# volume-em/empanada

Measured on AMD Instinct MI355X. Metric: Mvox/s end-to-end 3D panoptic inference (incl. consensus); PQ vs CPU ref, higher is better.
Workload: dtype f32

## Files before the change

### empanada_amd/csrc/emp_conv.hip

```cpp
#include "emp_common.h"
#include <stdlib.h>

typedef float f32x16 __attribute__((ext_vector_type(16)));

#define CG_BM 128
#define CG_BK 32
#define CG_THREADS 256

struct ConvGeom {
    const float *x, *w, *scale, *shift, *res;
    float *out;
    int N, H, W, Cin, OH, OW, Cout, KH, KW, stride, pad, dil, relu;
    int64_t M, out_ps, res_ps;
    int tiles_m, tiles_n;
    int64_t x_bs, w_bs, out_bs;
    const int32_t *tiles;
    const float *proj_w;
    float *proj_out;
    int proj_n;
    int64_t hw;
};

__device__ __attribute__((aligned(16))) float cg_zero_page[64];

// ... 408 lines not shown
                        *reinterpret_cast<float4 *>(g.out + p * g.out_ps + co) = make_float4(v[0], v[1], v[2], v[3]);
                    } else {
#pragma unroll
                        for (int e = 0; e < 4; ++e)
                            if (co + e < g.Cout) g.out[p * g.out_ps + co + e] = v[e];
                    }
                }
            }
            if constexpr (PROJ) {
                float ps[4] = {0.f, 0.f, 0.f, 0.f};
                if (valid && co + 3 < g.Cout) {
#pragma unroll
                    for (int q = 0; q < 4; ++q)
                        if (q < g.proj_n) {
                            const float4 wq = *reinterpret_cast<const float4 *>(g.proj_w + (int64_t)q * g.Cout + co);
                            ps[q] = __fadd_rn(__fadd_rn(__fadd_rn(__fmul_rn(v[0], wq.x), __fmul_rn(v[1], wq.y)),
                                                        __fmul_rn(v[2], wq.z)), __fmul_rn(v[3], wq.w));
                        }
                }
                *reinterpret_cast<float4 *>(&Cs[lrow_c * CLD + ccol]) = make_float4(ps[0], ps[1], ps[2], ps[3]);
            }
        }
        if constexpr (PROJ) {
            __syncthreads();
            for (int idx = tid; idx < EPI_ROWS * g.proj_n; idx += CG_THREADS) {
                const int row_l = idx / g.proj_n, q = idx - row_l * g.proj_n;
                const int64_t p = m0 + rd * EPI_ROWS + row_l;
                if (p < g.M) {
                    float t = Cs[row_l * CLD + q];
#pragma unroll 8
                    for (int j = 1; j < C4; ++j) t = __fadd_rn(t, Cs[row_l * CLD + 4 * j + q]);
                    const int64_t img = p / g.hw;
                    atomicAdd(g.proj_out + (img * g.proj_n + q) * g.hw + (p - img * g.hw), t);
                }
            }
        }
    }
}

struct CgPlan {
    bool narrow, respf, glds;
    int slab, tiles_m, tiles_n;
};

static CgPlan cg_plan(int64_t M, int Cout, int batch, bool has_res, bool res_vec_ok, bool may_split_n = true, int cin = 32)
{
    CgPlan p;
    const int64_t wide_blocks = emp_cdiv(M, CG_BM) * emp_cdiv(Cout, 128) * batch;
    p.narrow = Cout <= 64 || (Cout % 128 != 0 && Cout % 128 <= 64 && Cout < 512) || (may_split_n && wide_blocks < 256);
    p.tiles_m = (int)emp_cdiv(M, CG_BM);
    p.tiles_n = (int)emp_cdiv(Cout, p.narrow ? 64 : 128);
    static const char *fnarrow = getenv("EMP_CONV_NARROW");
    static const char *norespf = getenv("EMP_CONV_NO_RESPF");
    if (fnarrow && fnarrow[0] == '1') {
        p.narrow = true;
        p.tiles_n = (int)emp_cdiv(Cout, 64);
    }
    p.respf = has_res && res_vec_ok && Cout % (p.narrow ? 64 : 128) == 0 && !norespf;
    static const char *force = getenv("EMP_CONV_BK");
    const int64_t blocks = (int64_t)p.tiles_m * p.tiles_n * batch;
    p.slab = blocks > 512 ? 16 : 32;
    if (force && force[0] == '1') p.slab = 16;
    if (force && force[0] == '3') p.slab = 32;
    if (p.respf) p.slab = 32;
    if (cin % 32 != 0) {
        p.slab = 16;
        p.respf = false;
    }
    static const char *noglds = getenv("EMP_CONV_NO_GLDS");
    p.glds = !noglds;
    return p;
}

extern "C" int emp_conv_k_slab(int64_t M, int Cout, int batch, int has_residual)
{
    return cg_plan(M, Cout, batch, has_residual != 0, true).slab;
}

extern "C" int emp_conv_k_slab_cin(int64_t M, int Cout, int batch, int has_residual, int Cin)
{
    return cg_plan(M, Cout, batch, has_residual != 0, true, true, Cin).slab;
}

extern "C" int emp_conv1x1_ws_eligible(int64_t M, int Cin, int Cout, int KH, int KW, int stride, int pad, int relu);
extern "C" __attribute__((visibility("hidden"))) int emp_conv1x1_ws_launch(const float *x, const float *w, const float *scale, const float *shift,
                                     const float *res, int64_t res_ps, int relu, int64_t M, int Cin, int Cout,
                                     float *out, int64_t out_ps, void *stream);

extern "C" int emp_conv_k_slab_geom(int64_t M, int Cout, int has_residual, int Cin, int KH, int KW, int stride, int pad,
                                    int relu)
{
    if (emp_conv1x1_ws_eligible(M, Cin, Cout, KH, KW, stride, pad, relu)) return 64;
    return cg_plan(M, Cout, 1, has_residual != 0 && relu != 2, true, true, Cin).slab;
}

extern "C" int emp_conv_bn_act_nhwc(const float *x, const float *w_okkc, const float *scale, const float *shift,
                                    const float *residual, int64_t res_pixel_stride, int relu, int N, int H, int W,
                                    int Cin, int Cout, int KH, int KW, int stride, int pad, int dil, float *out,
                                    int64_t out_pixel_stride, void *stream)
{
    EMP_REQUIRE(x && w_okkc && out, "conv: null pointer");
    EMP_REQUIRE(N >= 0 && H > 0 && W > 0 && Cin > 0 && Cout > 0, "conv: bad shape");
    EMP_REQUIRE(Cin % 16 == 0, "conv: Cin %d must be a multiple of 16", Cin);
    EMP_REQUIRE(relu != 2 || residual, "conv: the gate epilogue (relu == 2) needs the gated tensor as residual");
    EMP_REQUIRE(KH >= 1 && KW >= 1 && KH <= 7 && KW <= 7 && stride >= 1 && dil >= 1 && pad >= 0, "conv: bad filter geometry");
    const int OH = (H + 2 * pad - dil * (KH - 1) - 1) / stride + 1;
    const int OW = (W + 2 * pad - dil * (KW - 1) - 1) / stride + 1;
    EMP_REQUIRE(OH > 0 && OW > 0, "conv: empty output");
    if (out_pixel_stride == 0) out_pixel_stride = Cout;
    if (res_pixel_stride == 0) res_pixel_stride = Cout;
    EMP_REQUIRE(out_pixel_stride >= Cout && res_pixel_stride >= Cout, "conv: bad pixel stride");
    EMP_REQUIRE(((reinterpret_cast<uintptr_t>(x) | reinterpret_cast<uintptr_t>(w_okkc)) & 15) == 0,
                "conv: x and w must be 16-byte aligned");
    EMP_REQUIRE(out != x, "conv: output cannot alias the input");
    if (N == 0) return EMP_OK;
    ConvGeom g;
    g.x = x; g.w = w_okkc; g.scale = scale; g.shift = shift; g.res = residual; g.out = out;
    g.N = N; g.H = H; g.W = W; g.Cin = Cin; g.OH = OH; g.OW = OW; g.Cout = Cout; g.KH = KH; g.KW = KW;
    g.stride = stride; g.pad = pad; g.dil = dil; g.relu = relu;
    g.M = (int64_t)N * OH * OW; g.out_ps = out_pixel_stride; g.res_ps = res_pixel_stride;
    g.x_bs = g.w_bs = g.out_bs = 0; g.tiles = nullptr; g.proj_w = nullptr; g.proj_out = nullptr; g.proj_n = 0; g.hw = 1;
    const bool res_vec_ok = (res_pixel_stride & 3) == 0 && (reinterpret_cast<uintptr_t>(residual) & 15) == 0;
    const bool io_vec_ok = res_vec_ok && (out_pixel_stride & 3) == 0 && (reinterpret_cast<uintptr_t>(out) & 15) == 0 &&
                           (!scale || (reinterpret_cast<uintptr_t>(scale) & 15) == 0) &&
                           (!shift || (reinterpret_cast<uintptr_t>(shift) & 15) == 0);
    if (io_vec_ok && scale && shift && emp_conv1x1_ws_eligible(g.M, Cin, Cout, KH, KW, stride, pad, relu))
        return emp_conv1x1_ws_launch(x, w_okkc, scale, shift, residual, res_pixel_stride, relu, g.M, Cin, Cout, out,
                                     out_pixel_stride, stream);
    const CgPlan pl = cg_plan(g.M, Cout, 1, residual != nullptr && relu != 2, res_vec_ok, true, Cin);
    const bool narrow = pl.narrow, respf = pl.respf, bk16 = pl.slab == 16;
    EMP_REQUIRE((int64_t)pl.tiles_m * pl.tiles_n < (1LL << 28), "conv: too many tiles");
    g.tiles_m = pl.tiles_m;
    g.tiles_n = pl.tiles_n;
    const int T = g.tiles_m * g.tiles_n;
    const int grid = 8 * ((T + 7) / 8);
#define CG_GO(NT_, RES_, BK_, GL_) hipLaunchKernelGGL((conv_igemm_f32_kernel<NT_, 0, RES_, BK_, false, GL_>), dim3(grid), dim3(CG_THREADS), 0, emp_stream(stream), g)
#define CG_GATE(NT_, BK_) hipLaunchKernelGGL((conv_igemm_f32_kernel<NT_, 0, false, BK_, false, true, true>), dim3(grid), dim3(CG_THREADS), 0, emp_stream(stream), g)
    if (relu == 2) {
        if (narrow) { if (bk16) CG_GATE(1, 16); else CG_GATE(1, 32); }
        else { if (bk16) CG_GATE(2, 16); else CG_GATE(2, 32); }
    } else if (narrow) {
        if (respf) { if (pl.glds) CG_GO(1, true, 32, true); else CG_GO(1, true, 32, false); }
        else if (pl.glds) { if (bk16) CG_GO(1, false, 16, true); else CG_GO(1, false, 32, true); }
        else { if (bk16) CG_GO(1, false, 16, false); else CG_GO(1, false, 32, false); }
    } else {
        if (respf) { if (pl.glds) CG_GO(2, true, 32, true); else CG_GO(2, true, 32, false); }
        else if (pl.glds) { if (bk16) CG_GO(2, false, 16, true); else CG_GO(2, false, 32, true); }
        else { if (bk16) CG_GO(2, false, 16, false); else CG_GO(2, false, 32, false); }
    }
#undef CG_GO
#undef CG_GATE
    EMP_CHECK_LAUNCH("emp_conv_bn_act_nhwc");
    return EMP_OK;
}

__global__ __launch_bounds__(256) void splitk_reduce_kernel(const float *__restrict__ work, int nz, int64_t M, int Cout,
                                                            const float *__restrict__ scale,
                                                            const float *__restrict__ shift,
                                                            const float *__restrict__ res, int64_t res_ps, int relu,
                                                            float *__restrict__ out, int64_t out_ps)
{
    const int C4 = Cout >> 2;
    const int64_t total = M * C4, plane = M * (int64_t)Cout;
    for (int64_t i = (int64_t)blockIdx.x * blockDim.x + threadIdx.x; i < total; i += (int64_t)gridDim.x * blockDim.x) {
        const int64_t p = i / C4;
        const int co = (int)(i - p * C4) * 4;
        const float *w = work + p * Cout + co;
        float4 t = *reinterpret_cast<const float4 *>(w);
        for (int z = 1; z < nz; ++z) {
            const float4 u = *reinterpret_cast<const float4 *>(w + z * plane);
            t.x = __fadd_rn(t.x, u.x); t.y = __fadd_rn(t.y, u.y); t.z = __fadd_rn(t.z, u.z); t.w = __fadd_rn(t.w, u.w);
        }
        float v[4] = {t.x, t.y, t.z, t.w};
#pragma unroll
        for (int e = 0; e < 4; ++e) {
            const float sc = scale ? scale[co + e] : 1.f, sh = shift ? shift[co + e] : 0.f;
            v[e] = __fadd_rn(__fmul_rn(v[e], sc), sh);
        }
        if (res) {
            const float4 r4 = *reinterpret_cast<const float4 *>(res + p * res_ps + co);
            v[0] = __fadd_rn(v[0], r4.x); v[1] = __fadd_rn(v[1], r4.y); v[2] = __fadd_rn(v[2], r4.z); v[3] = __fadd_rn(v[3], r4.w);
        }
        if (relu) {
#pragma unroll
            for (int e = 0; e < 4; ++e) v[e] = fmaxf(v[e], 0.f);
        }
        *reinterpret_cast<float4 *>(out + p * out_ps + co) = make_float4(v[0], v[1], v[2], v[3]);
    }
}

extern "C" int emp_conv_splitk_plan(int64_t M, int Cout, int Cin, int KH, int KW)
{
    if (M <= 0 || Cout <= 0 || Cin % 32 != 0 || Cout % 4 != 0) return 1;
    const CgPlan pl = cg_plan(M, Cout, 1, false, true, true, Cin);
    const int64_t tiles = (int64_t)pl.tiles_m * pl.tiles_n;
    const int S = KH * KW * (Cin / 32);
    if (tiles > 128) return 1;
    int64_t k = 256 / tiles;
    if (k > S / 4) k = S / 4;
    if (k > 32) k = 32;
    return k >= 2 ? (int)k : 1;
}

extern "C" int emp_conv_splitk_bn_act_nhwc(const float *x, const float *w_okkc, const float *scale, const float *shift,
                                           const float *residual, int64_t res_pixel_stride, int relu, int N, int H, int W,
                                           int Cin, int Cout, int KH, int KW, int stride, int pad, int dil, int k_splits,
                                           float *work, float *out, int64_t out_pixel_stride, void *stream)
{
    EMP_REQUIRE(x && w_okkc && out && work, "conv_splitk: null pointer");
    EMP_REQUIRE(N >= 0 && H > 0 && W > 0 && Cin > 0 && Cout > 0, "conv_splitk: bad shape");
    EMP_REQUIRE(Cin % 32 == 0 && Cout % 4 == 0, "conv_splitk: Cin %d must be a multiple of 32, Cout %d of 4", Cin, Cout);
    EMP_REQUIRE(relu == 0 || relu == 1, "conv_splitk: relu must be 0 or 1");
// ... 112 lines not shown
            dst[(1 * 4 + v) * ps] = W_ADD(tt[1][v], tt[2][v]);
            dst[(2 * 4 + v) * ps] = W_SUB(tt[2][v], tt[1][v]);
            dst[(3 * 4 + v) * ps] = W_SUB(tt[1][v], tt[3][v]);
        }
    }
}

__global__ __launch_bounds__(256) void wino_output_kernel(const float4 *__restrict__ Mw, const int32_t *__restrict__ tiles,
                                                          int64_t T, int H, int W, int Co4, int dil,
                                                          const float4 *__restrict__ scale, const float4 *__restrict__ shift,
                                                          int relu, float *__restrict__ out, int64_t out_ps)
{
    const int64_t total = T * Co4;
    for (int64_t i = (int64_t)blockIdx.x * blockDim.x + threadIdx.x; i < total; i += (int64_t)gridDim.x * blockDim.x) {
        const int c4 = (int)(i % Co4);
        const int64_t t = i / Co4;
        const int n = tiles[3 * t], oy = tiles[3 * t + 1] + dil, ox = tiles[3 * t + 2] + dil;
        const float4 *src = Mw + t * Co4 + c4;
        const int64_t ps = T * Co4;
        float4 m[4][4];
#pragma unroll
        for (int a = 0; a < 4; ++a)
#pragma unroll
            for (int b = 0; b < 4; ++b) m[a][b] = src[(a * 4 + b) * ps];
        float4 s[2][4];
#pragma unroll
        for (int b = 0; b < 4; ++b) {
            s[0][b] = W_ADD(W_ADD(m[0][b], m[1][b]), m[2][b]);
            s[1][b] = W_SUB(W_SUB(m[1][b], m[2][b]), m[3][b]);
        }
        float4 sc = make_float4(1.f, 1.f, 1.f, 1.f), sh = make_float4(0.f, 0.f, 0.f, 0.f);
        if (scale) sc = scale[c4];
        if (shift) sh = shift[c4];
#pragma unroll
        for (int a = 0; a < 2; ++a) {
            float4 yv[2];
            yv[0] = W_ADD(W_ADD(s[a][0], s[a][1]), s[a][2]);
            yv[1] = W_SUB(W_SUB(s[a][1], s[a][2]), s[a][3]);
#pragma unroll
            for (int b = 0; b < 2; ++b) {
                const int yy = oy + a * dil, xx = ox + b * dil;
                if (yy < H && xx < W) {
                    float4 v = yv[b];
                    if (scale) v = make_float4(__fmul_rn(v.x, sc.x), __fmul_rn(v.y, sc.y), __fmul_rn(v.z, sc.z), __fmul_rn(v.w, sc.w));
                    if (shift) v = W_ADD(v, sh);
                    if (relu) v = make_float4(fmaxf(v.x, 0.f), fmaxf(v.y, 0.f), fmaxf(v.z, 0.f), fmaxf(v.w, 0.f));
                    *reinterpret_cast<float4 *>(out + (((int64_t)n * H + yy) * W + xx) * out_ps + 4 * c4) = v;
                }
            }
        }
    }
}
#undef W_SUB
#undef W_ADD

extern "C" int emp_wino_input_transform(const float *x, int N, int H, int W, int C, int dil, const int32_t *tiles,
                                        int64_t T, float *V, void *stream)
{
    EMP_REQUIRE(x && tiles && V, "wino_input: null pointer");
    EMP_REQUIRE(N > 0 && H > 0 && W > 0 && C > 0 && C % 4 == 0 && dil >= 1 && T >= 0, "wino_input: bad shape");
    EMP_REQUIRE(((reinterpret_cast<uintptr_t>(x) | reinterpret_cast<uintptr_t>(V)) & 15) == 0, "wino_input: alignment");
    if (T == 0) return EMP_OK;
    hipLaunchKernelGGL(wino_input_kernel, dim3(emp_grid(T * (C / 4), 256, 16384)), dim3(256), 0, emp_stream(stream), x,
                       tiles, T, H, W, C / 4, dil, reinterpret_cast<float4 *>(V));
    EMP_CHECK_LAUNCH("emp_wino_input_transform");
    return EMP_OK;
}

extern "C" int emp_gemm_nt_batched(const float *A, const float *B, int batch, int64_t M, int N, int K, float *C,
                                   void *stream)
{
    EMP_REQUIRE(A && B && C, "gemm: null pointer");
    EMP_REQUIRE(batch >= 1 && batch <= 65535 && M >= 0 && M < (1LL << 31) && N > 0 && K > 0 && K % CG_BK == 0,
                "gemm: bad shape (K must be a multiple of %d)", CG_BK);
    EMP_REQUIRE(((reinterpret_cast<uintptr_t>(A) | reinterpret_cast<uintptr_t>(B)) & 15) == 0, "gemm: alignment");
    if (M == 0) return EMP_OK;
    ConvGeom g;
    g.x = A; g.w = B; g.scale = g.shift = g.res = nullptr; g.out = C;
    g.N = 1; g.H = 1; g.W = (int)M; g.Cin = K; g.OH = 1; g.OW = (int)M; g.Cout = N; g.KH = g.KW = 1;
    g.stride = 1; g.pad = 0; g.dil = 1; g.relu = 0;
    g.M = M; g.out_ps = N; g.res_ps = N;
    g.x_bs = M * K; g.w_bs = (int64_t)N * K; g.out_bs = M * N; g.tiles = nullptr; g.proj_w = nullptr; g.proj_out = nullptr; g.proj_n = 0; g.hw = 1;
    const CgPlan pl = cg_plan(M, N, batch, false, true);
    const bool narrow = pl.narrow, bk16 = pl.slab == 16;
    g.tiles_m = pl.tiles_m;
    g.tiles_n = pl.tiles_n;
    const int T = g.tiles_m * g.tiles_n;
    dim3 grid(8 * ((T + 7) / 8), batch);
#define CG_GOG(NT_, BK_, GL_) hipLaunchKernelGGL((conv_igemm_f32_kernel<NT_, 0, false, BK_, false, GL_>), grid, dim3(CG_THREADS), 0, emp_stream(stream), g)
    if (narrow) {
        if (pl.glds) { if (bk16) CG_GOG(1, 16, true); else CG_GOG(1, 32, true); }
        else { if (bk16) CG_GOG(1, 16, false); else CG_GOG(1, 32, false); }
    } else {
        if (pl.glds) { if (bk16) CG_GOG(2, 16, true); else CG_GOG(2, 32, true); }
        else { if (bk16) CG_GOG(2, 16, false); else CG_GOG(2, 32, false); }
    }
#undef CG_GOG
    EMP_CHECK_LAUNCH("emp_gemm_nt_batched");
    return EMP_OK;
}

extern "C" int emp_wino_gemm_fused(const float *x, int N, int H, int W, int Cin, int dil, const int32_t *tiles,
                                   int64_t T, const float *U, int Cout, float *Mw, void *stream)
{
    EMP_REQUIRE(x && tiles && U && Mw, "wino_gemm: null pointer");
    EMP_REQUIRE(N > 0 && H > 0 && W > 0 && Cin > 0 && Cin % CG_BK == 0 && Cout > 0 && dil >= 1 && T >= 0,
                "wino_gemm: bad shape (Cin must be a multiple of %d)", CG_BK);
    EMP_REQUIRE((int64_t)N * H * W * Cin < (1LL << 31) && T < (1LL << 31), "wino_gemm: activation too large for 32-bit offsets");
    EMP_REQUIRE(((reinterpret_cast<uintptr_t>(x) | reinterpret_cast<uintptr_t>(U)) & 15) == 0, "wino_gemm: alignment");
    if (T == 0) return EMP_OK;
    ConvGeom g;
    g.x = x; g.w = U; g.scale = g.shift = g.res = nullptr; g.out = Mw;
    g.N = N; g.H = H; g.W = W; g.Cin = Cin; g.OH = 1; g.OW = 1; g.Cout = Cout; g.KH = g.KW = 1;
    g.stride = 1; g.pad = 0; g.dil = dil; g.relu = 0;
    g.M = T; g.out_ps = Cout; g.res_ps = Cout;
    g.x_bs = 0; g.w_bs = (int64_t)Cout * Cin; g.out_bs = T * Cout; g.tiles = tiles; g.proj_w = nullptr; g.proj_out = nullptr; g.proj_n = 0; g.hw = 1;
    const bool narrow = Cout <= 64;
    g.tiles_m = (int)emp_cdiv(T, CG_BM);
    g.tiles_n = (int)emp_cdiv(Cout, narrow ? 64 : 128);
    const int nt = g.tiles_m * g.tiles_n;
    dim3 grid(8 * ((nt + 7) / 8), 16);
    if (narrow) hipLaunchKernelGGL((conv_igemm_f32_kernel<1, 1>), grid, dim3(CG_THREADS), 0, emp_stream(stream), g);
    else hipLaunchKernelGGL((conv_igemm_f32_kernel<2, 1>), grid, dim3(CG_THREADS), 0, emp_stream(stream), g);
    EMP_CHECK_LAUNCH("emp_wino_gemm_fused");
    return EMP_OK;
}

extern "C" int emp_wino_output_transform(const float *Mw, const int32_t *tiles, int64_t T, int N, int H, int W,
                                         int Cout, int dil, const float *scale, const float *shift, int relu,
                                         float *out, int64_t out_pixel_stride, void *stream)
{
    EMP_REQUIRE(Mw && tiles && out, "wino_output: null pointer");
    EMP_REQUIRE(N > 0 && H > 0 && W > 0 && Cout > 0 && Cout % 4 == 0 && dil >= 1 && T >= 0, "wino_output: bad shape");
    if (out_pixel_stride == 0) out_pixel_stride = Cout;
    EMP_REQUIRE(out_pixel_stride >= Cout && out_pixel_stride % 4 == 0, "wino_output: bad pixel stride");
    EMP_REQUIRE(((reinterpret_cast<uintptr_t>(Mw) | reinterpret_cast<uintptr_t>(out) | reinterpret_cast<uintptr_t>(scale) |
                  reinterpret_cast<uintptr_t>(shift)) & 15) == 0, "wino_output: alignment");
    if (T == 0) return EMP_OK;
    hipLaunchKernelGGL(wino_output_kernel, dim3(emp_grid(T * (Cout / 4), 256, 16384)), dim3(256), 0, emp_stream(stream),
                       reinterpret_cast<const float4 *>(Mw), tiles, T, H, W, Cout / 4, dil,
                       reinterpret_cast<const float4 *>(scale), reinterpret_cast<const float4 *>(shift), relu, out,
                       out_pixel_stride);
    EMP_CHECK_LAUNCH("emp_wino_output_transform");
    return EMP_OK;
}

struct v4 {
    float x, y, z, w;
};
__device__ __forceinline__ v4 operator+(v4 a, v4 b) { return {__fadd_rn(a.x, b.x), __fadd_rn(a.y, b.y), __fadd_rn(a.z, b.z), __fadd_rn(a.w, b.w)}; }
__device__ __forceinline__ v4 operator-(v4 a, v4 b) { return {__fsub_rn(a.x, b.x), __fsub_rn(a.y, b.y), __fsub_rn(a.z, b.z), __fsub_rn(a.w, b.w)}; }
__device__ __forceinline__ v4 operator*(float k, v4 a) { return {__fmul_rn(k, a.x), __fmul_rn(k, a.y), __fmul_rn(k, a.z), __fmul_rn(k, a.w)}; }
__device__ __forceinline__ v4 ldv4(const float4 *p) { float4 t = *p; return {t.x, t.y, t.z, t.w}; }
__device__ __forceinline__ void stv4(float4 *p, v4 a) { *p = make_float4(a.x, a.y, a.z, a.w); }

__device__ __forceinline__ void wino4_bt(const v4 d[6], v4 r[6])
{
    r[0] = (4.f * d[0] - 5.f * d[2]) + d[4];
    r[1] = (d[3] + d[4]) - 4.f * (d[1] + d[2]);
    r[2] = (d[4] - d[3]) + 4.f * (d[1] - d[2]);
    r[3] = (d[4] - d[2]) + 2.f * (d[3] - d[1]);
    r[4] = (d[4] - d[2]) + 2.f * (d[1] - d[3]);
    r[5] = (4.f * d[1] - 5.f * d[3]) + d[5];
}

__device__ __forceinline__ void wino4_at(const v4 m[6], v4 s[4])
// ... 262 lines not shown
```

### empanada_amd/csrc/emp_conv1x1.hip

```cpp
#include "emp_common.h"
#include <stdlib.h>

typedef float f32x16 __attribute__((ext_vector_type(16)));

#define PW_THREADS 256
#define PW_BN 128
#define PW_ROWS 32

struct PwGeom {
    const float *x, *w, *scale, *shift, *res;
    float *out;
    int64_t M, out_ps, res_ps;
    int Cin, Cout, relu, groups, pix_blocks;
};

template <int KS, bool RES, bool RELU>
__global__ __launch_bounds__(PW_THREADS, 1) void conv1x1_ws_kernel(PwGeom g)
{
    constexpr int CIN = 64 * KS;
    constexpr int LD = CIN + 4;
    __shared__ __attribute__((aligned(16))) float Bs[PW_BN * LD];

    const int bid = blockIdx.x;
    const int xcd = bid & 7, slot = bid >> 3;
    const int per_xcd = g.pix_blocks >> 3;
    const int gi = slot % g.groups;
    const int pb = xcd * per_xcd + slot / g.groups;
    const int n0 = gi * PW_BN;
    const int tid = threadIdx.x;

    for (int idx = tid; idx < PW_BN * (CIN / 4); idx += PW_THREADS) {
        const int rr = idx / (CIN / 4), k4 = idx - rr * (CIN / 4);
        const int co = n0 + 4 * (rr & 31) + (rr >> 5);
        *reinterpret_cast<float4 *>(&Bs[rr * LD + 4 * k4]) = *reinterpret_cast<const float4 *>(g.w + (int64_t)co * CIN + 4 * k4);
    }
    __syncthreads();

    const int wave = tid >> 6, lane = tid & 63;
    const int r = lane & 31, hh = lane >> 5;
    const int co = n0 + 4 * r;
    float sc[4], sh[4];
    { const float4 t = *reinterpret_cast<const float4 *>(g.scale + co); sc[0] = t.x; sc[1] = t.y; sc[2] = t.z; sc[3] = t.w; }
    { const float4 t = *reinterpret_cast<const float4 *>(g.shift + co); sh[0] = t.x; sh[1] = t.y; sh[2] = t.z; sh[3] = t.w; }

    const int64_t n_tiles = (g.M + PW_ROWS - 1) / PW_ROWS;
    const int64_t stride_t = (int64_t)g.pix_blocks * (PW_THREADS / 64);
    const float *Bl = &Bs[r * LD + hh * 32];

    auto load_a = [&](int64_t t, float4 (&a)[KS][8]) {
        const int64_t pa = t * PW_ROWS + r;
        const float *ap = g.x + pa * CIN + hh * 32;
#pragma unroll
        for (int s = 0; s < KS; ++s)
#pragma unroll
            for (int q = 0; q < 8; ++q) a[s][q] = *reinterpret_cast<const float4 *>(ap + 64 * s + 4 * q);
    };
    auto load_rs = [&](int64_t t, float4 (&rs)[RES ? 16 : 1]) {
        if constexpr (RES) {
            const float *rp = g.res + (t * PW_ROWS + 4 * hh) * g.res_ps + co;
#pragma unroll
            for (int q = 0; q < 16; ++q)
                rs[q] = *reinterpret_cast<const float4 *>(rp + (int64_t)((q & 3) + 8 * (q >> 2)) * g.res_ps);
        }
    };
    auto mma = [&](f32x16 (&acc)[4], const float4 (&a)[KS][8]) {
#pragma unroll
        for (int j = 0; j < 4; ++j)
#pragma unroll
            for (int q = 0; q < 16; ++q) acc[j][q] = 0.f;
        int opaque = 0;
        asm volatile("" : "+v"(opaque));
        const float *Bt = Bl + opaque;
#pragma unroll
        for (int s = 0; s < KS; ++s)
#pragma unroll
            for (int q = 0; q < 8; ++q) {
                float4 b[4];
#pragma unroll
                for (int j = 0; j < 4; ++j) b[j] = *reinterpret_cast<const float4 *>(Bt + j * 32 * LD + 64 * s + 4 * q);
#pragma unroll
                for (int e = 0; e < 4; ++e) {
                    const float av = e == 0 ? a[s][q].x : e == 1 ? a[s][q].y : e == 2 ? a[s][q].z : a[s][q].w;
#pragma unroll
                    for (int j = 0; j < 4; ++j) {
                        const float bv = e == 0 ? b[j].x : e == 1 ? b[j].y : e == 2 ? b[j].z : b[j].w;
                        acc[j] = __builtin_amdgcn_mfma_f32_32x32x2f32(av, bv, acc[j], 0, 0, 0);
                    }
                }
            }
    };
    auto outv = [&](const f32x16 (&acc)[4], const float4 (&rs)[RES ? 16 : 1], int q) {
        float v[4] = {acc[0][q], acc[1][q], acc[2][q], acc[3][q]};
#pragma unroll
        for (int e = 0; e < 4; ++e) v[e] = __fadd_rn(__fmul_rn(v[e], sc[e]), sh[e]);
        if constexpr (RES) {
            v[0] = __fadd_rn(v[0], rs[q].x); v[1] = __fadd_rn(v[1], rs[q].y);
            v[2] = __fadd_rn(v[2], rs[q].z); v[3] = __fadd_rn(v[3], rs[q].w);
        }
        if constexpr (RELU) {
#pragma unroll
            for (int e = 0; e < 4; ++e) v[e] = fmaxf(v[e], 0.f);
        }
        return make_float4(v[0], v[1], v[2], v[3]);
    };
    auto epi = [&](const f32x16 (&acc)[4], const float4 (&rs)[RES ? 16 : 1], int64_t t) {
        float *op = g.out + (t * PW_ROWS + 4 * hh) * g.out_ps + co;
#pragma unroll
        for (int q = 0; q < 16; ++q)
            *reinterpret_cast<float4 *>(op + (int64_t)((q & 3) + 8 * (q >> 2)) * g.out_ps) = outv(acc, rs, q);
    };

    const int64_t n_full = g.M / PW_ROWS;
    const int64_t t_first = (int64_t)pb * (PW_THREADS / 64) + wave;
    if (t_first < n_full) {
        const int64_t m = (n_full - t_first + stride_t - 1) / stride_t;
        auto tile = [&](int64_t i) { return t_first + (i < m ? i : m - 1) * stride_t; };
        float4 a0[KS][8], a1[KS][8], rs0[RES ? 16 : 1], rs1[RES ? 16 : 1];
        f32x16 acc0[4], acc1[4];
        load_a(tile(0), a0);
        load_rs(tile(0), rs0);
        load_a(tile(1), a1);
        mma(acc0, a0);
        int64_t i = 1;
        for (; i + 1 < m; i += 2) {
            load_rs(tile(i), rs1);
            load_a(tile(i + 1), a0);
            mma(acc1, a1);
            epi(acc0, rs0, tile(i - 1));
            load_rs(tile(i + 1), rs0);
            load_a(tile(i + 2), a1);
            mma(acc0, a0);
            epi(acc1, rs1, tile(i));
        }
        if (i < m) {
            load_rs(tile(i), rs1);
            mma(acc1, a1);
            epi(acc0, rs0, tile(i - 1));
            epi(acc1, rs1, tile(i));
        } else {
            epi(acc0, rs0, tile(i - 1));
        }
    }
    if (n_full < n_tiles && (n_full - t_first) % stride_t == 0 && n_full >= t_first) {
        const int64_t p0 = n_full * PW_ROWS;
        const int64_t pa = (p0 + r < g.M) ? p0 + r : g.M - 1;
        const float *ap = g.x + pa * CIN + hh * 32;
        float4 a[KS][8], rs[RES ? 16 : 1];
        f32x16 acc[4];
#pragma unroll
        for (int s = 0; s < KS; ++s)
#pragma unroll
            for (int q = 0; q < 8; ++q) a[s][q] = *reinterpret_cast<const float4 *>(ap + 64 * s + 4 * q);
        if constexpr (RES) {
#pragma unroll
            for (int q = 0; q < 16; ++q) {
                int64_t p = p0 + (q & 3) + 8 * (q >> 2) + 4 * hh;
                p = p < g.M ? p : g.M - 1;
                rs[q] = *reinterpret_cast<const float4 *>(g.res + p * g.res_ps + co);
            }
        }
        mma(acc, a);
#pragma unroll
        for (int q = 0; q < 16; ++q) {
            const int64_t p = p0 + (q & 3) + 8 * (q >> 2) + 4 * hh;
            if (p < g.M) *reinterpret_cast<float4 *>(g.out + p * g.out_ps + co) = outv(acc, rs, q);
        }
    }
}

extern "C" int emp_conv1x1_ws_eligible(int64_t M, int Cin, int Cout, int KH, int KW, int stride, int pad, int relu)
{
    static const char *off = getenv("EMP_CONV_NO_WS");
    if (off && off[0] == '1') return 0;
    return KH == 1 && KW == 1 && stride == 1 && pad == 0 && (Cin == 64 || Cin == 128) && Cout % PW_BN == 0 &&
           Cout / PW_BN <= 8 && relu != 2 && M >= 65536;
}

extern "C" __attribute__((visibility("hidden"))) int emp_conv1x1_ws_launch(const float *x, const float *w, const float *scale, const float *shift,
                                     const float *res, int64_t res_ps, int relu, int64_t M, int Cin, int Cout,
                                     float *out, int64_t out_ps, void *stream)
{
    PwGeom g;
    g.x = x; g.w = w; g.scale = scale; g.shift = shift; g.res = res; g.out = out;
    g.M = M; g.out_ps = out_ps; g.res_ps = res_ps; g.Cin = Cin; g.Cout = Cout; g.relu = relu;
    g.groups = Cout / PW_BN;
    int pix = 256 / g.groups;
    pix = pix / 8 * 8;
    if (pix < 8) pix = 8;
    g.pix_blocks = pix;
    const dim3 grid(pix * g.groups), block(PW_THREADS);
    hipStream_t st = emp_stream(stream);
#define PW_GO(KS_, RES_, RELU_) hipLaunchKernelGGL((conv1x1_ws_kernel<KS_, RES_, RELU_>), grid, block, 0, st, g)
#define PW_GO2(KS_, RES_) do { if (relu) PW_GO(KS_, RES_, true); else PW_GO(KS_, RES_, false); } while (0)
    if (Cin == 64) { if (res) PW_GO2(1, true); else PW_GO2(1, false); }
    else { if (res) PW_GO2(2, true); else PW_GO2(2, false); }
#undef PW_GO2
#undef PW_GO
    EMP_CHECK_LAUNCH("emp_conv_bn_act_nhwc(1x1 weight-stationary)");
    return EMP_OK;
}
```

Before: 127.6.

## Extend weight-stationary 1x1 kernel to narrow Cout, wide Cin, and batched GEMM

Generalizes the weight-stationary pointwise MFMA kernel with templated K-slab, Cout tile width (64 or 128) and pixel-tile count. It now covers extra 1x1 conv shapes (256->64, 64->64, 256->128) where the planner picks a 16-wide slab, and the batched NT GEMM path for K and N of 64 or 128. The GEMM mode splits batch×tiles evenly across 256 blocks and restages weights per batch segment. The aim is to replace the generic implicit-GEMM kernel on these large shapes, avoiding repeated weight reloads. The cost is more template instantiations, and K-slab orderings that differ from the old path may slightly change summation order.

Measured after the change: 129.5 (median of 6 runs). 1.02x the previous value.

```diff
diff --git a/empanada_amd/csrc/emp_conv.hip b/empanada_amd/csrc/emp_conv.hip
--- a/empanada_amd/csrc/emp_conv.hip
+++ b/empanada_amd/csrc/emp_conv.hip
@@ -514,15 +514,18 @@
     return cg_plan(M, Cout, batch, has_residual != 0, true, true, Cin).slab;
 }
 
-extern "C" int emp_conv1x1_ws_eligible(int64_t M, int Cin, int Cout, int KH, int KW, int stride, int pad, int relu);
-extern "C" __attribute__((visibility("hidden"))) int emp_conv1x1_ws_launch(const float *x, const float *w, const float *scale, const float *shift,
+extern "C" __attribute__((visibility("hidden"))) int emp_conv1x1_ws_kind(int64_t M, int Cin, int Cout, int KH, int KW, int stride, int pad, int relu);
+extern "C" __attribute__((visibility("hidden"))) int emp_conv1x1_ws_launch(int kind, const float *x, const float *w, const float *scale, const float *shift,
                                      const float *res, int64_t res_ps, int relu, int64_t M, int Cin, int Cout,
                                      float *out, int64_t out_ps, void *stream);
+extern "C" __attribute__((visibility("hidden"))) int emp_gemm_ws_eligible(int batch, int64_t M, int N, int K, int slab);
+extern "C" __attribute__((visibility("hidden"))) int emp_gemm_ws_launch(const float *A, const float *B, int batch, int64_t M, int N, int K, float *C,
+                                                                        void *stream);
 
 extern "C" int emp_conv_k_slab_geom(int64_t M, int Cout, int has_residual, int Cin, int KH, int KW, int stride, int pad,
                                     int relu)
 {
-    if (emp_conv1x1_ws_eligible(M, Cin, Cout, KH, KW, stride, pad, relu)) return 64;
+    if (emp_conv1x1_ws_kind(M, Cin, Cout, KH, KW, stride, pad, relu) == 1) return 64;
     return cg_plan(M, Cout, 1, has_residual != 0 && relu != 2, true, true, Cin).slab;
 }
 
@@ -556,10 +559,14 @@
     const bool io_vec_ok = res_vec_ok && (out_pixel_stride & 3) == 0 && (reinterpret_cast<uintptr_t>(out) & 15) == 0 &&
                            (!scale || (reinterpret_cast<uintptr_t>(scale) & 15) == 0) &&
                            (!shift || (reinterpret_cast<uintptr_t>(shift) & 15) == 0);
-    if (io_vec_ok && scale && shift && emp_conv1x1_ws_eligible(g.M, Cin, Cout, KH, KW, stride, pad, relu))
-        return emp_conv1x1_ws_launch(x, w_okkc, scale, shift, residual, res_pixel_stride, relu, g.M, Cin, Cout, out,
+    const int ws = io_vec_ok && scale && shift ? emp_conv1x1_ws_kind(g.M, Cin, Cout, KH, KW, stride, pad, relu) : 0;
+    if (ws == 1)
+        return emp_conv1x1_ws_launch(1, x, w_okkc, scale, shift, residual, res_pixel_stride, relu, g.M, Cin, Cout, out,
                                      out_pixel_stride, stream);
     const CgPlan pl = cg_plan(g.M, Cout, 1, residual != nullptr && relu != 2, res_vec_ok, true, Cin);
+    if (ws == 2 && !residual && pl.slab == 16)
+        return emp_conv1x1_ws_launch(2, x, w_okkc, scale, shift, nullptr, res_pixel_stride, relu, g.M, Cin, Cout, out,
+                                     out_pixel_stride, stream);
     const bool narrow = pl.narrow, respf = pl.respf, bk16 = pl.slab == 16;
     EMP_REQUIRE((int64_t)pl.tiles_m * pl.tiles_n < (1LL << 28), "conv: too many tiles");
     g.tiles_m = pl.tiles_m;
@@ -838,6 +845,8 @@
     g.M = M; g.out_ps = N; g.res_ps = N;
     g.x_bs = M * K; g.w_bs = (int64_t)N * K; g.out_bs = M * N; g.tiles = nullptr; g.proj_w = nullptr; g.proj_out = nullptr; g.proj_n = 0; g.hw = 1;
     const CgPlan pl = cg_plan(M, N, batch, false, true);
+    if ((reinterpret_cast<uintptr_t>(C) & 15) == 0 && emp_gemm_ws_eligible(batch, M, N, K, pl.slab))
+        return emp_gemm_ws_launch(A, B, batch, M, N, K, C, stream);
     const bool narrow = pl.narrow, bk16 = pl.slab == 16;
     g.tiles_m = pl.tiles_m;
     g.tiles_n = pl.tiles_n;
diff --git a/empanada_amd/csrc/emp_conv1x1.hip b/empanada_amd/csrc/emp_conv1x1.hip
--- a/empanada_amd/csrc/emp_conv1x1.hip
+++ b/empanada_amd/csrc/emp_conv1x1.hip
@@ -4,198 +4,298 @@
 typedef float f32x16 __attribute__((ext_vector_type(16)));
 
 #define PW_THREADS 256
-#define PW_BN 128
 #define PW_ROWS 32
+#define PW_MIN_ROWS 65536
+#define PW_MIN_ROWS_PLAN 262144
 
 struct PwGeom {
     const float *x, *w, *scale, *shift, *res;
     float *out;
     int64_t M, out_ps, res_ps;
     int Cin, Cout, relu, groups, pix_blocks;
+    int batch;
+    int64_t x_bs, w_bs, out_bs;
 };
 
-template <int KS, bool RES, bool RELU>
+template <int KS, int S, int CT, int PT, bool GEMM, bool RES, bool RELU>
 __global__ __launch_bounds__(PW_THREADS, 1) void conv1x1_ws_kernel(PwGeom g)
 {
     constexpr int CIN = 64 * KS;
     constexpr int LD = CIN + 4;
-    __shared__ __attribute__((aligned(16))) float Bs[PW_BN * LD];
+    constexpr int BN = 32 * CT;
+    constexpr int NQ = CIN / 8;
+    constexpr int QS = S / 8;
+    constexpr int ROWS = PW_ROWS * PT;
+    static_assert(!RES || (CT == 4 && PT == 1 && !GEMM), "residual: 128-cout groups of the convolution form only");
+    static_assert(S == 16 || S == 32 || S == 64, "K-slab");
+    __shared__ __attribute__((aligned(16))) float Bs[BN * LD];
 
     const int bid = blockIdx.x;
     const int xcd = bid & 7, slot = bid >> 3;
     const int per_xcd = g.pix_blocks >> 3;
     const int gi = slot % g.groups;
     const int pb = xcd * per_xcd + slot / g.groups;
-    const int n0 = gi * PW_BN;
+    const int n0 = GEMM ? 0 : gi * BN;
     const int tid = threadIdx.x;
-
-    for (int idx = tid; idx < PW_BN * (CIN / 4); idx += PW_THREADS) {
-        const int rr = idx / (CIN / 4), k4 = idx - rr * (CIN / 4);
-        const int co = n0 + 4 * (rr & 31) + (rr >> 5);
-        *reinterpret_cast<float4 *>(&Bs[rr * LD + 4 * k4]) = *reinterpret_cast<const float4 *>(g.w + (int64_t)co * CIN + 4 * k4);
-    }
-    __syncthreads();
+    const float *xb = g.x, *wb = g.w;
+    float *ob = g.out;
+
+    auto stage = [&]() {
+        for (int idx = tid; idx < BN * (CIN / 4); idx += PW_THREADS) {
+            const int rr = idx / (CIN / 4), k4 = idx - rr * (CIN / 4);
+            const int cw = n0 + CT * (rr & 31) + (rr >> 5);
+            *reinterpret_cast<float4 *>(&Bs[rr * LD + 4 * k4]) = *reinterpret_cast<const float4 *>(wb + (int64_t)cw * CIN + 4 * k4);
+        }
+        __syncthreads();
+    };
 
     const int wave = tid >> 6, lane = tid & 63;
     const int r = lane & 31, hh = lane >> 5;
-    const int co = n0 + 4 * r;
-    float sc[4], sh[4];
-    { const float4 t = *reinterpret_cast<const float4 *>(g.scale + co); sc[0] = t.x; sc[1] = t.y; sc[2] = t.z; sc[3] = t.w; }
-    { const float4 t = *reinterpret_cast<const float4 *>(g.shift + co); sh[0] = t.x; sh[1] = t.y; sh[2] = t.z; sh[3] = t.w; }
-
-    const int64_t n_tiles = (g.M + PW_ROWS - 1) / PW_ROWS;
-    const int64_t stride_t = (int64_t)g.pix_blocks * (PW_THREADS / 64);
-    const float *Bl = &Bs[r * LD + hh * 32];
-
-    auto load_a = [&](int64_t t, float4 (&a)[KS][8]) {
-        const int64_t pa = t * PW_ROWS + r;
-        const float *ap = g.x + pa * CIN + hh * 32;
-#pragma unroll
-        for (int s = 0; s < KS; ++s)
-#pragma unroll
-            for (int q = 0; q < 8; ++q) a[s][q] = *reinterpret_cast<const float4 *>(ap + 64 * s + 4 * q);
+    const int co = n0 + CT * r;
+    float sc[CT], sh[CT];
+    if constexpr (!GEMM) {
+        if constexpr (CT == 4) {
+            { const float4 t = *reinterpret_cast<const float4 *>(g.scale + co); sc[0] = t.x; sc[1] = t.y; sc[2] = t.z; sc[3] = t.w; }
+            { const float4 t = *reinterpret_cast<const float4 *>(g.shift + co); sh[0] = t.x; sh[1] = t.y; sh[2] = t.z; sh[3] = t.w; }
+        } else {
+            { const float2 t = *reinterpret_cast<const float2 *>(g.scale + co); sc[0] = t.x; sc[1] = t.y; }
+            { const float2 t = *reinterpret_cast<const float2 *>(g.shift + co); sh[0] = t.x; sh[1] = t.y; }
+        }
+    }
+
+    const int64_t n_tiles = (g.M + ROWS - 1) / ROWS;
+    const int64_t n_full = g.M / ROWS;
+    const float *Bl = &Bs[r * LD + hh * (S / 2)];
+    const int64_t ops = GEMM ? (int64_t)BN : g.out_ps;
+
+    auto load_a = [&](int64_t t, float4 (&a)[PT][NQ]) {
+#pragma unroll
+        for (int p = 0; p < PT; ++p) {
+            const int64_t pa = t * ROWS + PW_ROWS * p + r;
+            const float *ap = xb + pa * CIN + hh * (S / 2);
+#pragma unroll
+            for (int i = 0; i < NQ; ++i) a[p][i] = *reinterpret_cast<const float4 *>(ap + S * (i / QS) + 4 * (i % QS));
+        }
     };
     auto load_rs = [&](int64_t t, float4 (&rs)[RES ? 16 : 1]) {
         if constexpr (RES) {
-            const float *rp = g.res + (t * PW_ROWS + 4 * hh) * g.res_ps + co;
+            const float *rp = g.res + (t * ROWS + 4 * hh) * g.res_ps + co;
 #pragma unroll
             for (int q = 0; q < 16; ++q)
                 rs[q] = *reinterpret_cast<const float4 *>(rp + (int64_t)((q & 3) + 8 * (q >> 2)) * g.res_ps);
         }
     };
-    auto mma = [&](f32x16 (&acc)[4], const float4 (&a)[KS][8]) {
-#pragma unroll
-        for (int j = 0; j < 4; ++j)
+    auto mma = [&](f32x16 (&acc)[PT * CT], const float4 (&a)[PT][NQ]) {
+#pragma unroll
+        for (int j = 0; j < PT * CT; ++j)
 #pragma unroll
             for (int q = 0; q < 16; ++q) acc[j][q] = 0.f;
         int opaque = 0;
         asm volatile("" : "+v"(opaque));
         const float *Bt = Bl + opaque;
 #pragma unroll
-        for (int s = 0; s < KS; ++s)
-#pragma unroll
-            for (int q = 0; q < 8; ++q) {
-                float4 b[4];
-#pragma unroll
-                for (int j = 0; j < 4; ++j) b[j] = *reinterpret_cast<const float4 *>(Bt + j * 32 * LD + 64 * s + 4 * q);
-#pragma unroll
-                for (int e = 0; e < 4; ++e) {
-                    const float av = e == 0 ? a[s][q].x : e == 1 ? a[s][q].y : e == 2 ? a[s][q].z : a[s][q].w;
-#pragma unroll
-                    for (int j = 0; j < 4; ++j) {
+        for (int i = 0; i < NQ; ++i) {
+            float4 b[CT];
+#pragma unroll
+            for (int j = 0; j < CT; ++j) b[j] = *reinterpret_cast<const float4 *>(Bt + j * 32 * LD + S * (i / QS) + 4 * (i % QS));
+#pragma unroll
+            for (int e = 0; e < 4; ++e)
+#pragma unroll
+                for (int p = 0; p < PT; ++p) {
+                    const float av = e == 0 ? a[p][i].x : e == 1 ? a[p][i].y : e == 2 ? a[p][i].z : a[p][i].w;
+#pragma unroll
+                    for (int j = 0; j < CT; ++j) {
                         const float bv = e == 0 ? b[j].x : e == 1 ? b[j].y : e == 2 ? b[j].z : b[j].w;
-                        acc[j] = __builtin_amdgcn_mfma_f32_32x32x2f32(av, bv, acc[j], 0, 0, 0);
+                        acc[p * CT + j] = __builtin_amdgcn_mfma_f32_32x32x2f32(av, bv, acc[p * CT + j], 0, 0, 0);
                     }
                 }
-            }
-    };
-    auto outv = [&](const f32x16 (&acc)[4], const float4 (&rs)[RES ? 16 : 1], int q) {
-        float v[4] = {acc[0][q], acc[1][q], acc[2][q], acc[3][q]};
-#pragma unroll
-        for (int e = 0; e < 4; ++e) v[e] = __fadd_rn(__fmul_rn(v[e], sc[e]), sh[e]);
+        }
+    };
+    auto put = [&](float *dst, const f32x16 (&acc)[PT * CT], int p, const float4 (&rs)[RES ? 16 : 1], int q) {
+        float v[CT];
+#pragma unroll
+        for (int e = 0; e < CT; ++e) v[e] = acc[p * CT + e][q];
+        if constexpr (!GEMM) {
+#pragma unroll
+            for (int e = 0; e < CT; ++e) v[e] = __fadd_rn(__fmul_rn(v[e], sc[e]), sh[e]);
+        }
         if constexpr (RES) {
             v[0] = __fadd_rn(v[0], rs[q].x); v[1] = __fadd_rn(v[1], rs[q].y);
             v[2] = __fadd_rn(v[2], rs[q].z); v[3] = __fadd_rn(v[3], rs[q].w);
         }
         if constexpr (RELU) {
 #pragma unroll
-            for (int e = 0; e < 4; ++e) v[e] = fmaxf(v[e], 0.f);
-        }
-        return make_float4(v[0], v[1], v[2], v[3]);
-    };
-    auto epi = [&](const f32x16 (&acc)[4], const float4 (&rs)[RES ? 16 : 1], int64_t t) {
-        float *op = g.out + (t * PW_ROWS + 4 * hh) * g.out_ps + co;
-#pragma unroll
-        for (int q = 0; q < 16; ++q)
-            *reinterpret_cast<float4 *>(op + (int64_t)((q & 3) + 8 * (q >> 2)) * g.out_ps) = outv(acc, rs, q);
-    };
-
-    const int64_t n_full = g.M / PW_ROWS;
-    const int64_t t_first = (int64_t)pb * (PW_THREADS / 64) + wave;
-    if (t_first < n_full) {
-        const int64_t m = (n_full - t_first + stride_t - 1) / stride_t;
-        auto tile = [&](int64_t i) { return t_first + (i < m ? i : m - 1) * stride_t; };
-        float4 a0[KS][8], a1[KS][8], rs0[RES ? 16 : 1], rs1[RES ? 16 : 1];
-        f32x16 acc0[4], acc1[4];
-        load_a(tile(0), a0);
-        load_rs(tile(0), rs0);
-        load_a(tile(1), a1);
-        mma(acc0, a0);
-        int64_t i = 1;
-        for (; i + 1 < m; i += 2) {
-            load_rs(tile(i), rs1);
-            load_a(tile(i + 1), a0);
-            mma(acc1, a1);
-            epi(acc0, rs0, tile(i - 1));
-            load_rs(tile(i + 1), rs0);
-            load_a(tile(i + 2), a1);
+            for (int e = 0; e < CT; ++e) v[e] = fmaxf(v[e], 0.f);
+        }
+        if constexpr (CT == 4) *reinterpret_cast<float4 *>(dst) = make_float4(v[0], v[1], v[2], v[3]);
+        else *reinterpret_cast<float2 *>(dst) = make_float2(v[0], v[1]);
+    };
+    auto epi = [&](const f32x16 (&acc)[PT * CT], const float4 (&rs)[RES ? 16 : 1], int64_t t) {
+#pragma unroll
+        for (int p = 0; p < PT; ++p) {
+            float *op = ob + (t * ROWS + PW_ROWS * p + 4 * hh) * ops + co;
+#pragma unroll
+            for (int q = 0; q < 16; ++q) put(op + (int64_t)((q & 3) + 8 * (q >> 2)) * ops, acc, p, rs, q);
+        }
+    };
+
+    auto run = [&](const int64_t t_first, const int64_t stride_t, const int64_t t_end) {
+        const int64_t f_end = n_full < t_end ? n_full : t_end;
+        if (t_first < f_end) {
+            const int64_t m = (f_end - t_first + stride_t - 1) / stride_t;
+            auto tile = [&](int64_t i) { return t_first + (i < m ? i : m - 1) * stride_t; };
+            float4 a0[PT][NQ], a1[PT][NQ], rs0[RES ? 16 : 1], rs1[RES ? 16 : 1];
+            f32x16 acc0[PT * CT], acc1[PT * CT];
+            load_a(tile(0), a0);
+            load_rs(tile(0), rs0);
+            load_a(tile(1), a1);
             mma(acc0, a0);
-            epi(acc1, rs1, tile(i));
-        }
-        if (i < m) {
-            load_rs(tile(i), rs1);
-            mma(acc1, a1);
-            epi(acc0, rs0, tile(i - 1));
-            epi(acc1, rs1, tile(i));
-        } else {
-            epi(acc0, rs0, tile(i - 1));
-        }
+            int64_t i = 1;
+            for (; i + 1 < m; i += 2) {
+                load_rs(tile(i), rs1);
+                load_a(tile(i + 1), a0);
+                mma(acc1, a1);
+                epi(acc0, rs0, tile(i - 1));
+                load_rs(tile(i + 1), rs0);
+                load_a(tile(i + 2), a1);
+                mma(acc0, a0);
+                epi(acc1, rs1, tile(i));
+            }
+            if (i < m) {
+                load_rs(tile(i), rs1);
+                mma(acc1, a1);
+                epi(acc0, rs0, tile(i - 1));
+                epi(acc1, rs1, tile(i));
+            } else {
+                epi(acc0, rs0, tile(i - 1));
+            }
+        }
+        if (n_full < t_end && n_full >= t_first && (n_full - t_first) % stride_t == 0) {
+            const int64_t p0 = n_full * ROWS;
+            float4 a[PT][NQ], rs[RES ? 16 : 1];
+            f32x16 acc[PT * CT];
+#pragma unroll
+            for (int p = 0; p < PT; ++p) {
+                const int64_t pr = p0 + PW_ROWS * p + r;
+                const float *ap = xb + (pr < g.M ? pr : g.M - 1) * CIN + hh * (S / 2);
+#pragma unroll
+                for (int i = 0; i < NQ; ++i) a[p][i] = *reinterpret_cast<const float4 *>(ap + S * (i / QS) + 4 * (i % QS));
+            }
+            if constexpr (RES) {
+#pragma unroll
+                for (int q = 0; q < 16; ++q) {
+                    int64_t p = p0 + (q & 3) + 8 * (q >> 2) + 4 * hh;
+                    p = p < g.M ? p : g.M - 1;
+                    rs[q] = *reinterpret_cast<const float4 *>(g.res + p * g.res_ps + co);
+                }
+            }
+            mma(acc, a);
+#pragma unroll
+            for (int p = 0; p < PT; ++p)
+#pragma unroll
+                for (int q = 0; q < 16; ++q) {
+                    const int64_t px = p0 + PW_ROWS * p + (q & 3) + 8 * (q >> 2) + 4 * hh;
+                    if (px < g.M) put(ob + px * ops + co, acc, p, rs, q);
+                }
+        }
+    };
+
+    if constexpr (GEMM) {
+        const int64_t G = (int64_t)g.batch * n_tiles;
+        int64_t lo = G * bid / gridDim.x;
+        const int64_t hi = G * (bid + 1) / gridDim.x;
+        while (lo < hi) {
+            const int64_t b = lo / n_tiles, t0 = lo - b * n_tiles;
+            const int64_t t1 = hi - lo < n_tiles - t0 ? t0 + (hi - lo) : n_tiles;
+            xb = g.x + b * g.x_bs;
+            wb = g.w + b * g.w_bs;
+            ob = g.out + b * g.out_bs;
+            stage();
+            run(t0 + wave, PW_THREADS / 64, t1);
+            __syncthreads();
+            lo += t1 - t0;
+        }
+    } else {
+        stage();
+        run((int64_t)pb * (PW_THREADS / 64) + wave, (int64_t)g.pix_blocks * (PW_THREADS / 64), n_tiles);
     }
-    if (n_full < n_tiles && (n_full - t_first) % stride_t == 0 && n_full >= t_first) {
-        const int64_t p0 = n_full * PW_ROWS;
-        const int64_t pa = (p0 + r < g.M) ? p0 + r : g.M - 1;
-        const float *ap = g.x + pa * CIN + hh * 32;
-        float4 a[KS][8], rs[RES ? 16 : 1];
-        f32x16 acc[4];
-#pragma unroll
-        for (int s = 0; s < KS; ++s)
-#pragma unroll
-            for (int q = 0; q < 8; ++q) a[s][q] = *reinterpret_cast<const float4 *>(ap + 64 * s + 4 * q);
-        if constexpr (RES) {
-#pragma unroll
-            for (int q = 0; q < 16; ++q) {
-                int64_t p = p0 + (q & 3) + 8 * (q >> 2) + 4 * hh;
-                p = p < g.M ? p : g.M - 1;
-                rs[q] = *reinterpret_cast<const float4 *>(g.res + p * g.res_ps + co);
-            }
-        }
-        mma(acc, a);
-#pragma unroll
-        for (int q = 0; q < 16; ++q) {
-            const int64_t p = p0 + (q & 3) + 8 * (q >> 2) + 4 * hh;
-            if (p < g.M) *reinterpret_cast<float4 *>(g.out + p * g.out_ps + co) = outv(acc, rs, q);
-        }
+}
+
+static bool pw_off()
+{
+    static const char *off = getenv("EMP_CONV_NO_WS");
+    return off && off[0] == '1';
+}
+
+extern "C" __attribute__((visibility("hidden"))) int emp_conv1x1_ws_kind(int64_t M, int Cin, int Cout, int KH, int KW, int stride, int pad, int relu)
+{
+    if (pw_off()) return 0;
+    if (!(KH == 1 && KW == 1 && stride == 1 && pad == 0 && relu != 2)) return 0;
+    if ((Cin == 64 || Cin == 128) && Cout % 128 == 0 && Cout / 128 <= 8 && M >= PW_MIN_ROWS) return 1;
+    if (M >= PW_MIN_ROWS_PLAN && ((Cin == 256 && Cout == 64) || (Cin == 64 && Cout == 64) || (Cin == 256 && Cout == 128)))
+        return 2;
+    return 0;
+}
+
+extern "C" int emp_conv1x1_ws_eligible(int64_t M, int Cin, int Cout, int KH, int KW, int stride, int pad, int relu)
+{
+    return emp_conv1x1_ws_kind(M, Cin, Cout, KH, KW, stride, pad, relu) != 0;
+}
+
+extern "C" __attribute__((visibility("hidden"))) int emp_gemm_ws_eligible(int batch, int64_t M, int N, int K, int slab)
+{
+    if (pw_off()) return 0;
+    return (K == 64 || K == 128) && (N == 64 || N == 128) && slab == 16 && M >= PW_ROWS && (int64_t)batch * M >= PW_MIN_ROWS_PLAN;
+}
+
+template <int KS, int S, int CT, int PT, bool GEMM, bool RES>
+static void pw_go(const PwGeom &g, int blocks, hipStream_t st)
+{
+    if (g.relu) {
+        if constexpr (!GEMM) hipLaunchKernelGGL((conv1x1_ws_kernel<KS, S, CT, PT, GEMM, RES, true>), dim3(blocks), dim3(PW_THREADS), 0, st, g);
+    } else {
+        hipLaunchKernelGGL((conv1x1_ws_kernel<KS, S, CT, PT, GEMM, RES, false>), dim3(blocks), dim3(PW_THREADS), 0, st, g);
     }
 }
 
-extern "C" int emp_conv1x1_ws_eligible(int64_t M, int Cin, int Cout, int KH, int KW, int stride, int pad, int relu)
-{
-    static const char *off = getenv("EMP_CONV_NO_WS");
-    if (off && off[0] == '1') return 0;
-    return KH == 1 && KW == 1 && stride == 1 && pad == 0 && (Cin == 64 || Cin == 128) && Cout % PW_BN == 0 &&
-           Cout / PW_BN <= 8 && relu != 2 && M >= 65536;
-}
-
-extern "C" __attribute__((visibility("hidden"))) int emp_conv1x1_ws_launch(const float *x, const float *w, const float *scale, const float *shift,
+extern "C" __attribute__((visibility("hidden"))) int emp_conv1x1_ws_launch(int kind, const float *x, const float *w, const float *scale, const float *shift,
                                      const float *res, int64_t res_ps, int relu, int64_t M, int Cin, int Cout,
                                      float *out, int64_t out_ps, void *stream)
 {
     PwGeom g;
     g.x = x; g.w = w; g.scale = scale; g.shift = shift; g.res = res; g.out = out;
     g.M = M; g.out_ps = out_ps; g.res_ps = res_ps; g.Cin = Cin; g.Cout = Cout; g.relu = relu;
-    g.groups = Cout / PW_BN;
+    g.batch = 1; g.x_bs = g.w_bs = g.out_bs = 0;
+    g.groups = kind == 1 ? Cout / 128 : 1;
     int pix = 256 / g.groups;
     pix = pix / 8 * 8;
     if (pix < 8) pix = 8;
     g.pix_blocks = pix;
-    const dim3 grid(pix * g.groups), block(PW_THREADS);
+    const int blocks = pix * g.groups;
     hipStream_t st = emp_stream(stream);
-#define PW_GO(KS_, RES_, RELU_) hipLaunchKernelGGL((conv1x1_ws_kernel<KS_, RES_, RELU_>), grid, block, 0, st, g)
-#define PW_GO2(KS_, RES_) do { if (relu) PW_GO(KS_, RES_, true); else PW_GO(KS_, RES_, false); } while (0)
-    if (Cin == 64) { if (res) PW_GO2(1, true); else PW_GO2(1, false); }
-    else { if (res) PW_GO2(2, true); else PW_GO2(2, false); }
-#undef PW_GO2
-#undef PW_GO
+    if (kind == 1) {
+        if (Cin == 64) { if (res) pw_go<1, 64, 4, 1, false, true>(g, blocks, st); else pw_go<1, 64, 4, 1, false, false>(g, blocks, st); }
+        else { if (res) pw_go<2, 64, 4, 1, false, true>(g, blocks, st); else pw_go<2, 64, 4, 1, false, false>(g, blocks, st); }
+    } else {
+        if (Cin == 64) pw_go<1, 16, 2, 2, false, false>(g, blocks, st);
+        else if (Cout == 64) pw_go<4, 16, 2, 1, false, false>(g, blocks, st);
+        else pw_go<4, 16, 4, 1, false, false>(g, blocks, st);
+    }
     EMP_CHECK_LAUNCH("emp_conv_bn_act_nhwc(1x1 weight-stationary)");
     return EMP_OK;
 }
+
+extern "C" __attribute__((visibility("hidden"))) int emp_gemm_ws_launch(const float *A, const float *B, int batch, int64_t M, int N, int K, float *C,
+                                                                        void *stream)
+{
+    PwGeom g;
+    g.x = A; g.w = B; g.scale = g.shift = g.res = nullptr; g.out = C;
+    g.M = M; g.out_ps = N; g.res_ps = N; g.Cin = K; g.Cout = N; g.relu = 0;
+    g.batch = batch; g.x_bs = M * K; g.w_bs = (int64_t)N * K; g.out_bs = M * N;
+    g.groups = 1; g.pix_blocks = 256;
+    hipStream_t st = emp_stream(stream);
+    if (K == 64) { if (N == 64) pw_go<1, 16, 2, 2, true, false>(g, 256, st); else pw_go<1, 16, 4, 1, true, false>(g, 256, st); }
+    else { if (N == 64) pw_go<2, 16, 2, 2, true, false>(g, 256, st); else pw_go<2, 16, 4, 1, true, false>(g, 256, st); }
+    EMP_CHECK_LAUNCH("emp_gemm_nt_batched(weight-stationary)");
+    return EMP_OK;
+}
```
